# kvignesh1420/rlap

Hardware: AMD Instinct MI355X
Metric: eliminated-vertices/sec (higher is better)
Workload: dtype f64

## Files before the change

__graft_entry__.py:

```python
import os
import subprocess
import sys

ROOT = os.path.dirname(os.path.abspath(__file__))
if ROOT not in sys.path:
    sys.path.insert(0, ROOT)


def build() -> None:
    subprocess.check_call(["make", "-C", os.path.join(ROOT, "rlap_amd", "csrc"), "-s", "ARCH=gfx950"])
    subprocess.check_call(["make", "-C", os.path.join(ROOT, "oracle"), "-s"])
    src = os.path.join(ROOT, "tests", "csrc", "host_mirror.cc")
    so = os.path.join(ROOT, "tests", "csrc", "libhost_mirror.so")
    subprocess.check_call(["g++", "-std=c++17", "-O2", "-msse4.2", "-mavx", "-fPIC", "-shared", "-o", so, src])
    src16 = os.path.join(ROOT, "tests", "csrc", "host_mirror_narrow.cc")
    so16 = os.path.join(ROOT, "tests", "csrc", "libhost_mirror_narrow.so")
    subprocess.check_call(["g++", "-std=c++17", "-O2", "-msse4.2", "-mavx", "-fPIC", "-shared", "-o", so16, src16])
    subprocess.check_call(["gcc", "-std=c99", "-Wall", "-Wextra", "-O1", "-I", os.path.join(ROOT, "include"), "-I", "/opt/rocm/include",
                           os.path.join(ROOT, "examples", "cabi_caller.c"), "-o", os.path.join(ROOT, "examples", "cabi_caller"),
                           "-L", os.path.join(ROOT, "rlap_amd"), "-lrlap_hip", "-L", "/opt/rocm/lib", "-lamdhip64",
                           "-Wl,-rpath,$ORIGIN/../rlap_amd", "-Wl,-rpath,/opt/rocm/lib"])
    import rlap_amd
    from rlap_amd import _lib
    _lib.load()


def smoke() -> None:
    import numpy as np
    import torch
    assert torch.cuda.is_available(), "smoke() needs cuda:0"
    import oracle
    from rlap_amd import graphs, ops
    n = 2000
    ei = graphs.barabasi_albert(n, 8, 1)
    with torch.cuda.device(0):
        out = ops.approximate_cholesky(ei.cuda(), None, n, n // 2, "degree", "asc").numpy()
    ref = oracle.approximate_cholesky(ei.numpy(), None, n, n // 2, "degree", "asc")
    assert out.shape == ref.shape and np.array_equal(out, ref), "HIP path differs from the oracle"
    perm = np.random.RandomState(0).permutation(n)
    with torch.cuda.device(0):
        out2 = ops.approximate_cholesky(ei.cuda(), None, n, n // 2, "random", "asc", perm=torch.from_numpy(perm)).numpy()
    ref2 = oracle.approximate_cholesky(ei.numpy(), None, n, n // 2, "random", "asc", perm=perm)
    assert out2.shape == ref2.shape and np.array_equal(out2, ref2), "HIP path differs from the oracle (o_v=random)"
    print(f"smoke ok: {out.shape[0]} rows bit-exact vs oracle; stats={ops.last_stats}")


if __name__ == "__main__":
    build()
    if len(sys.argv) > 1 and sys.argv[1] == "smoke":
        smoke()
```

rlap_amd/csrc/rlap_core.h:

```cpp
#pragma once
#include <stdint.h>

#if defined(__HIPCC__)
#define RLAP_HD __host__ __device__ __forceinline__
#define RLAP_HD_NOINLINE __host__ __device__ __noinline__
#else
#define RLAP_HD inline
#define RLAP_HD_NOINLINE inline
#endif

namespace rlap {

enum { OV_RANDOM = 0, OV_DEGREE = 1, OV_COARSEN = 2 };
enum { ON_ASC = 0, ON_DESC = 1, ON_RANDOM = 2 };

enum {
    ST_OK = 0,
    ST_NOT_SYMMETRIC = 1,
    ST_INDEX_RANGE = 2,
    ST_BAD_ARG = 3,
    ST_POOL_OVERFLOW = 4,
    ST_LOG_OVERFLOW = 5,
    ST_RNG_OVERFLOW = 6,
    ST_OUT_OVERFLOW = 7,
// ... 471 lines not shown
            for (int32_t j = 0; j < m; ++j) { csum += B.a_val[j]; B.cum[j] = csum; }
            if (A.rng_mode != RNG_COUNTER && G.n_draws >= A.rng_len) return ST_RNG_OVERFLOW;
            double u = arr_uniform(A, G.n_draws, v, 0); G.n_draws += 1;
            double r = u * csum;
            int32_t koff = upper_index(B.cum, m, r);
            int32_t k = B.a_nbr[koff];
            double wk = B.a_val[koff];
            A.e[B.a_twin[koff]].val = 0;
            int32_t xk = B.t_of[koff];
            pq_op(B.t_key[xk], B.t_mv[xk], G.n, -1, len0);
            for (int32_t j = 0; j < m; ++j) {
                if (j == koff) continue;
                pq_op(B.t_key[xk], B.t_mv[xk], G.n, +1, len0 + 1 + j);
                double w = B.a_val[j];
                double nw = (wk * w) / (wk + w);
                int rc = serial_rewire(A, B.a_twin[j], B.a_nbr[j], k, nw);
                if (rc) return rc;
            }
        }
    } else {
        double csum = 0;
        for (int32_t j = 0; j < m; ++j) { csum += B.a_val[j]; B.cum[j] = csum; }
        if (A.rng_mode != RNG_COUNTER && m > 1 && G.n_draws + (m - 1) > A.rng_len) return ST_RNG_OVERFLOW;
        double wdeg = csum, colScale = 1;
        for (int32_t j = 0; j < m - 1; ++j) {
            double w = B.a_val[j] * colScale;
            double f = w / wdeg;
            double u = arr_uniform(A, G.n_draws + j, v, j);
            double r = u * (csum - B.cum[j]) + B.cum[j];
            int32_t koff = upper_index(B.cum, m, r);
            B.ksel[j] = koff;
            double omf = 1 - f;
            B.newv[j] = f * omf * wdeg;
            colScale = colScale * omf;
            wdeg = wdeg * omf * omf;
        }
        if (m > 1) G.n_draws += m - 1;
        for (int32_t j = 0; j < m - 1; ++j) {
            int32_t koff = B.ksel[j];
            if (use_pq) { int32_t xk = B.t_of[koff]; pq_op(B.t_key[xk], B.t_mv[xk], G.n, +1, len0 + j); }
            int rc = serial_rewire(A, B.a_twin[j], B.a_nbr[j], B.a_nbr[koff], B.newv[j]);
            if (rc) return rc;
        }
        if (m > 0) {
            if (use_pq && e1 + 1 < (int64_t)G.n) { int32_t xl = B.t_of[m - 1]; pq_op(B.t_key[xl], B.t_mv[xl], G.n, -1, len0 + m); }
            A.e[B.a_twin[m - 1]].val = 0;
        }
    }
    if (use_pq) return pq_commit_serial(A, G, B, m);
    return ST_OK;
}

RLAP_HD int32_t serial_output(const Arrays& A, const GraphDesc& G, const ColBuf& B, int32_t cap, int32_t v, double* out, int64_t row0, bool count_only) {
    int32_t len0 = serial_gather(A, v, B, cap);
    if (len0 > cap) return -1;
    int32_t m = serial_sort_merge(A, G, B, len0, false, false);
    if (count_only) return m;
    serial_order(A, B, m, v, 1, G.vbase);
    for (int32_t j = 0; j < m; ++j) {
        double* o = out + 3 * (row0 + j);
        o[0] = (double)B.a_nbr[j]; o[1] = (double)v; o[2] = B.a_val[j];
    }
    return m;
}


constexpr int BCAP = 32;

struct TRes {
    int32_t key_after;
    int16_t mv;
    uint8_t c;
    uint8_t flags;
};
struct Ent {
    double val;
    union {
        double aux;
        TRes res;
    };
    int32_t nbr;
    int32_t twin;
};
enum { CF_BIG = 1, CF_DUP = 2, CF_COMPLEX = 4, CF_DEP = 8, CF_TIE = 16, CF_NEQ = 32, CF_READY = 64, CF_PATCHED = 128 };
constexpr int DEPMAX = 4;
enum { TF_CONTENDED = 1 };

template <int BC> struct CandPad {};
template <> struct CandPad<64> { int64_t pad64; };
template <> struct CandPad<128> { int64_t pad128; };
template <int BC>
struct CandT : CandPad<BC> {
    static constexpr int CAP = BC;
    Ent e[BC];
    uint8_t ksel[BC];
    int32_t v;
    int32_t m;
    int32_t flags;
    int32_t src;
    int32_t ndraw;
    int32_t koff;
    int32_t cp1;
    int32_t acnt;
    int32_t ext;
    int32_t nmv;
    int32_t nkill;
    int32_t cb[BC <= 16 ? 2 : (BC <= 32 ? 3 : (BC <= 64 ? 4 : 5))];
    int32_t ndep;
    uint8_t dep[4];
    int64_t draw0;
};
static_assert(sizeof(CandT<16>) == 472 && sizeof(CandT<32>) == 872, "record sizes the LDS budget of the round kernel is counted with");
typedef CandT<BCAP> Cand;

RLAP_HD TRes& ent_tres(Ent& e) { return e.res; }

struct EntLessNbr { RLAP_HD bool operator()(const Ent& x, const Ent& y) const { return x.nbr < y.nbr; } };
struct EntLessVal { RLAP_HD bool operator()(const Ent& x, const Ent& y) const { return x.val < y.val; } };
struct EntGreaterVal { RLAP_HD bool operator()(const Ent& x, const Ent& y) const { return x.val > y.val; } };
struct EntLessAux { RLAP_HD bool operator()(const Ent& x, const Ent& y) const { return x.aux < y.aux; } };

struct KI { double k; uint8_t idx; };
struct KIRef {
    Ent* e; uint8_t* ix; int i;
    RLAP_HD operator KI() const { KI v; v.k = e[i].aux; v.idx = ix[i]; return v; }
    RLAP_HD KIRef& operator=(const KI& v) { e[i].aux = v.k; ix[i] = v.idx; return *this; }
    RLAP_HD KIRef& operator=(const KIRef& o) { KI v = o; e[i].aux = v.k; ix[i] = v.idx; return *this; }
};
struct KIArr {
    Ent* e; uint8_t* ix;
    RLAP_HD KIRef operator[](int i) const { KIRef r; r.e = e; r.ix = ix; r.i = i; return r; }
};
struct KILess { RLAP_HD bool operator()(const KI& x, const KI& y) const { return x.k < y.k; } };
struct KIGreater { RLAP_HD bool operator()(const KI& x, const KI& y) const { return x.k > y.k; } };

template <class CT>
RLAP_HD void cand_order_index(const Arrays& A, CT& C) {
    const int32_t m = C.m;
    for (int32_t j = 0; j < m; ++j) C.ksel[j] = (uint8_t)j;
    KIArr arr; arr.e = C.e; arr.ix = C.ksel;
    if (CT::CAP <= 32) {
        if (A.o_n == ON_DESC && A.o_v != OV_COARSEN) gs_std_sort_small<KI>(arr, m, KIGreater());
        else gs_std_sort_small<KI>(arr, m, KILess());
    } else {
        if (A.o_n == ON_DESC && A.o_v != OV_COARSEN) gs_std_sort<KI>(arr, m, KIGreater());
        else gs_std_sort<KI>(arr, m, KILess());
    }
    C.ndraw = (A.o_v == OV_COARSEN) ? (m >= 1 ? 1 : 0) : (m > 1 ? m - 1 : 0);
}

template <class CT>
RLAP_HD bool cand_merges_multi_edges(const Arrays& A) { return CT::CAP >= 64 && A.o_v == OV_RANDOM; }

template <class CT>
RLAP_HD void cand_meta(const Arrays& A, int32_t v, CT& C) {
    C.v = v; C.flags = 0; C.m = 0; C.ndraw = 0; C.koff = 0; C.nkill = 0; C.nmv = 0; C.ndep = 0;
    int32_t cp0 = A.colptr[v], cp1 = A.colptr[v + 1];
    int32_t acnt = A.vr[v].app_cnt;
    int32_t base = A.vr[v].app_chunk;
    C.cp1 = cp1; C.acnt = acnt; C.ext = (cp1 - cp0) + acnt;
    if (C.ext > CT::CAP) { C.flags = CF_BIG; C.ext = 0; return; }
    if (acnt > 0) {
        int ct = chunk_of(acnt - 1);
        for (int c = ct; c >= 0; --c) { C.cb[c] = base; if (c > 0) base = A.e[base].nbr; }
    }
}
template <class CT>
RLAP_HD int32_t cand_slot(const CT& C, int32_t e) {
    if (e < C.acnt) {
        int32_t a = C.acnt - 1 - e;
        int c = chunk_of(a);
        return C.cb[c] + 1 + (a - chunk_start(c));
    }
    return C.cp1 - 1 - (e - C.acnt);
}
template <class CT>
RLAP_HD void cand_load(const Arrays& A, CT& C, int32_t e) {
    int32_t s = cand_slot(C, e);
    C.e[e].val = A.e[s].val; C.e[e].nbr = A.e[s].nbr; C.e[e].twin = A.e[s].twin; C.e[e].aux = 0;
}
template <class CT>
RLAP_HD void cand_finish(const Arrays& A, CT& C, int32_t vbase = 0) {
    if (C.flags & CF_BIG) return;
    int32_t len = 0;
    for (int32_t e = 0; e < C.ext; ++e) {
        if (C.e[e].val > 0) { if (len != e) C.e[len] = C.e[e]; ++len; }
    }
    C.m = len;
    gs_std_sort<Ent>(C.e, len, EntLessNbr());
    if (cand_merges_multi_edges<CT>(A)) {
        int32_t mm = 0, nk = 0;
        int32_t kill[CT::CAP];
        for (int32_t i = 0; i < len; ++i) {
            if (mm == 0 || C.e[i].nbr != C.e[mm - 1].nbr) { if (mm != i) C.e[mm] = C.e[i]; ++mm; }
            else { C.e[mm - 1].val += C.e[i].val; kill[nk++] = C.e[i].twin; }
        }
        for (int32_t q = 0; q < nk; ++q) C.e[mm + q].twin = kill[q];
        C.nkill = nk;
        len = mm;
        C.m = len;
    } else {
        for (int32_t i = 1; i < len; ++i) if (C.e[i].nbr == C.e[i - 1].nbr) { C.flags = CF_DUP; return; }
    }
    if (A.o_n == ON_RANDOM || A.o_v == OV_COARSEN) {
        uint64_t kb = keyed_order_base(A.shuffle_seed, C.v - vbase, 0);
        for (int32_t i = 0; i < len; ++i) C.e[i].aux = keyed_order_dkey(kb, C.e[i].nbr - vbase);
        gs_std_sort<Ent>(C.e, len, EntLessAux());
    } else if (A.o_n == ON_ASC) {
        gs_std_sort<Ent>(C.e, len, EntLessVal());
    } else {
        gs_std_sort<Ent>(C.e, len, EntGreaterVal());
    }
    C.ndraw = (A.o_v == OV_COARSEN) ? (len >= 1 ? 1 : 0) : (len > 1 ? len - 1 : 0);
}
template <class CT>
RLAP_HD void cand_prepare(const Arrays& A, int32_t v, CT& C, int32_t vbase = 0) {
    cand_meta(A, v, C);
    for (int32_t e = 0; e < C.ext; ++e) cand_load(A, C, e);
    cand_finish(A, C, vbase);
}

template <class CT>
RLAP_HD bool cand_patch(const Arrays& A, CT* cand, int32_t d, int32_t vbase) {
    CT& C = cand[d];
    if (C.nkill > 0) return false;
    for (int32_t q = 0; q < C.ndep; ++q) {
        const int32_t j = C.dep[q];
        const CT& J = cand[j];
        int32_t p = -1;
        for (int32_t z = 0; z < J.m; ++z) if (J.e[z].nbr == C.v) p = z;
        if (p < 0 || p == J.m - 1) return false;
        for (int32_t z = 0; z < J.m - 1; ++z) if (J.ksel[z] == p) return false;
        if (!(J.e[p].val > 0)) return false;
        const int32_t k = J.e[J.ksel[p]].nbr;
        int32_t qd = -1;
        for (int32_t z = 0; z < C.m; ++z) { if (C.e[z].nbr == J.v) qd = z; if (C.e[z].nbr == k) { C.flags |= CF_DUP; return false; } }
        if (qd < 0) return false;
        C.e[qd].nbr = k; C.e[qd].val = J.e[p].val; C.e[qd].twin = ~(j * CT::CAP + p);
    }
    C.flags |= CF_PATCHED;
    const int32_t len = C.m;
    gs_std_sort<Ent>(C.e, len, EntLessNbr());
    if (A.o_n == ON_RANDOM || A.o_v == OV_COARSEN) {
        uint64_t kb = keyed_order_base(A.shuffle_seed, C.v - vbase, 0);
        for (int32_t i = 0; i < len; ++i) C.e[i].aux = keyed_order_dkey(kb, C.e[i].nbr - vbase);
        gs_std_sort<Ent>(C.e, len, EntLessAux());
    } else if (A.o_n == ON_ASC) {
        gs_std_sort<Ent>(C.e, len, EntLessVal());
    } else {
        gs_std_sort<Ent>(C.e, len, EntGreaterVal());
    }
    return true;
}

RLAP_HD int32_t ent_upper_index(const Ent* e, int32_t m, double r) {
    int32_t lo = 0, hi = m;
    while (lo < hi) {
        int32_t mid = (lo + hi) >> 1;
        if (e[mid].aux > r) hi = mid; else lo = mid + 1;
    }
    return lo < m ? lo : m - 1;
}

template <class CT>
RLAP_HD void cand_cumsum(const Arrays& A, CT& C) {
    const int32_t m = C.m;
    double csum = 0;
    for (int32_t j = 0; j < m; ++j) { csum += C.e[j].val; C.e[j].aux = csum; }
    if (A.o_v == OV_COARSEN && m >= 1) {
        double u = arr_uniform(A, C.draw0, C.v, 0);
        double r = u * csum;
        int32_t koff = ent_upper_index(C.e, m, r);
        C.koff = koff;
        double wk = C.e[koff].val;
        for (int32_t j = 0; j < m; ++j) {
            if (j == koff) continue;
            double w = C.e[j].val;
            C.e[j].val = (wk * w) / (wk + w);
            C.ksel[j] = (uint8_t)koff;
        }
    }
}
template <class CT>
RLAP_HD void cand_pick(const Arrays& A, CT& C, int32_t j) {
    const int32_t m = C.m;
    double csum = C.e[m - 1].aux;
    double u = arr_uniform(A, C.draw0 + j, C.v, j);
    double cj = C.e[j].aux;
    double r = u * (csum - cj) + cj;
    C.ksel[j] = (uint8_t)ent_upper_index(C.e, m, r);
}
template <class CT>
RLAP_HD void cand_recur(const Arrays& A, CT& C) {
    if (A.o_v == OV_COARSEN) return;
    const int32_t m = C.m;
    if (m < 1) return;
    double wdeg = C.e[m - 1].aux, colScale = 1;
    for (int32_t j = 0; j < m - 1; ++j) {
        double w = C.e[j].val * colScale;
        double f = w / wdeg;
        double omf = 1 - f;
// ... 88 lines not shown
```

rlap_amd/csrc/rlap_kernels.hip:

```cpp
#include <hip/hip_runtime.h>
#include <stdint.h>
#include <cstdlib>
#include <type_traits>

#include "rlap_core.h"
#include "rlap_kernels.h"
#include "rlap_wave_sort.h"

namespace rlap {


#ifndef RLAP_ELIM_PQ_TU
__global__ __launch_bounds__(320) void k_mt19937_64_table(double* __restrict__ out, int64_t count) {
    constexpr int NN = 312, MM = 156;
    constexpr uint64_t MATRIX_A = 0xB5026F5AA96619E9ull, UM = 0xFFFFFFFF80000000ull, LM = 0x7FFFFFFFull;
    __shared__ uint64_t x[NN];
    const int tid = threadIdx.x;
    if (tid == 0) {
        uint64_t s = 5489ull;
        x[0] = s;
        for (int i = 1; i < NN; ++i) { s = 6364136223846793005ull * (s ^ (s >> 62)) + (uint64_t)i; x[i] = s; }
    }
    __syncthreads();
    for (int64_t base = 0; base < count; base += NN) {
// ... 863 lines not shown
        __hip_atomic_store(&help[0], 4, __ATOMIC_RELAXED, __HIP_MEMORY_SCOPE_WORKGROUP);
    }
#define BIG_HELP_FINISH() do { if (helped) { if (lane == 0) { int _sp = 0; while (__hip_atomic_load(&help[0], __ATOMIC_RELAXED, __HIP_MEMORY_SCOPE_WORKGROUP) != 2 && ++_sp < SPIN_LIMIT) __builtin_amdgcn_s_sleep(1); \
        if (_sp >= SPIN_LIMIT) G.status = ST_INTERNAL; \
        __hip_atomic_store(&help[0], 0, __ATOMIC_RELAXED, __HIP_MEMORY_SCOPE_WORKGROUP); } __builtin_amdgcn_fence(__ATOMIC_ACQUIRE, "workgroup"); WAVE_SYNC(); } \
        else if (lane == 0) __hip_atomic_store(&help[0], 3, __ATOMIC_RELAXED, __HIP_MEMORY_SCOPE_WORKGROUP); } while (0)
    if (lane == 0) {
        double csum = 0;
        for (int j = 0; j < m; ++j) { csum += cum[j]; cum[j] = csum; }
        if (!helped) {
            double wdeg = csum, colScale = 1;
            for (int j = 0; j < m - 1; ++j) {
                double w = newv[j] * colScale;
                double f = w / wdeg;
                double omf = 1 - f;
                newv[j] = f * omf * wdeg;
                colScale = colScale * omf;
                wdeg = wdeg * omf * omf;
            }
        }
    }
    WAVE_SYNC();
    const double csum = m > 0 ? cum[m - 1] : 0.0;
    const int64_t draws0 = G.n_draws;
    const int ndraw = m > 1 ? m - 1 : 0;
    if (draws0 + ndraw > A.rng_len) { BIG_HELP_FINISH(); if (lane == 0) G.status = ST_RNG_OVERFLOW; WAVE_SYNC(); return true; }

    for (int j = lane; j < m - 1; j += 64) {
        double u = arr_uniform(A, draws0 + j, v, j);
        double cj = cum[j];
        double r = u * (csum - cj) + cj;
        B.ksel[j] = upper_index(cum, m, r);
    }
    WAVE_SYNC();

    BIG_HELP_FINISH();
#undef BIG_HELP_FINISH
    int32_t status = 0;
    for (int j0 = 0; j0 < m - 1; j0 += 64) {
        const int j = j0 + lane;
        const bool act = j < m - 1;
        const int32_t ks = act ? B.ksel[j] : 0;
        const int32_t k = act ? B.a_nbr[ks] : -1;
        uint64_t mymask = __ballot(act);
        static_assert(BIGE <= 8192, "13 bits of target position");
#pragma unroll
        for (int bit = 0; bit < 13; ++bit) {
            const bool mybit = (ks >> bit) & 1;
            const uint64_t bb = __ballot(act && mybit);
            mymask &= mybit ? bb : ~bb;
        }
        if (act && lane == __builtin_ctzll(mymask)) {
            int32_t a = ld_agent(&A.vr[k].app_cnt), chunk = ld_agent(&A.vr[k].app_chunk);
            uint64_t mm = mymask;
            while (mm) { const int l = __builtin_ctzll(mm); mm &= mm - 1; L.tmp[l] = alloc_in_column(A, a, chunk, &status); }
            A.vr[k].app_cnt = a; A.vr[k].app_chunk = chunk;
        }
        __threadfence();
        WAVE_SYNC();
        if (act && status == 0) {
            const int32_t s_r = B.a_twin[j], s_n = L.tmp[lane];
            const double nw = newv[j];
            A.e[s_r].nbr = k; A.e[s_r].val = nw; A.e[s_r].twin = s_n;
            A.e[s_n].nbr = B.a_nbr[j]; A.e[s_n].val = nw; A.e[s_n].twin = s_r;
        }
        WAVE_SYNC();
        if (__ballot(status != 0) != 0ull) break;
    }
    if (__ballot(status != 0) != 0ull) { if (lane == 0) G.status = ST_POOL_OVERFLOW; WAVE_SYNC(); return true; }
    if (lane == 0) {
        if (m >= 1) A.e[B.a_twin[m - 1]].val = 0;
        G.n_draws = draws0 + ndraw;
    }
    WAVE_SYNC();
    return true;
}


constexpr int PASSES = 4;

struct CRec { int32_t x, i, j; };
constexpr int batch_ccap(int BC, int NTT) { return BC == 16 ? NTT / 4 : NTT / 2; }

template <int BC, int NTT>
struct BatchLdsT {
    CandT<BC> cand[4 * NTT / BC];
    union {
        struct {
            uint64_t mkey[NTT];
            int32_t mval[NTT];
            int32_t hidx[NTT];
        };
        int32_t hcnt[4 * NTT];
    };
    int32_t pslot[4 * NTT];
    unsigned long long cmask[4 * NTT / BC];
    CRec cont[batch_ccap(BC, NTT)];
    CRec csorted[batch_ccap(BC, NTT)];
    int32_t scan[NTT / 64 + 8];
};

template <int BC, int NTT>
union ElimSharedT {
    BatchLdsT<BC, NTT> b;
    ElimLdsT<(NTT >= 1024 ? ECAP : ECAP_SMALL)> e;
    BigElimLdsT<(NTT >= 1024 ? 7168 : 1536)> g;
};
static_assert(sizeof(ElimSharedT<64, 1024>) == sizeof(BatchLdsT<64, 1024>) && sizeof(ElimSharedT<32, 1024>) == sizeof(BatchLdsT<32, 1024>) &&
              sizeof(ElimSharedT<16, 1024>) == sizeof(BatchLdsT<16, 1024>),
              "the single-vertex paths borrow the batch round's LDS");

template <int NWAVE>
__device__ __noinline__ int block_excl_scan(int val, int* scratch, int* total) {
    const int tid = threadIdx.x, lane = tid & 63, wave = tid >> 6;
    int incl = val;
    for (int off = 1; off < 64; off <<= 1) { int t = __shfl_up(incl, off); if (lane >= off) incl += t; }
    if (lane == 63) scratch[wave] = incl;
    __syncthreads();
    int base = 0, tot = 0;
    for (int w = 0; w < NWAVE; ++w) { int sw = scratch[w]; if (w < wave) base += sw; tot += sw; }
    __syncthreads();
    *total = tot;
    return base + incl - val;
}

template <int NWAVE>
__device__ __forceinline__ int block_rank(bool flag, int* scratch, int* total) {
    return block_excl_scan<NWAVE>(flag ? 1 : 0, scratch, total);
}


__device__ __forceinline__ void rewire_store(const Arrays& A, int32_t s_r, int32_t s_n, int32_t nbr_j, int32_t k, double nw) {
    Slot a; a.val = nw; a.nbr = k; a.twin = s_n;
    Slot b; b.val = nw; b.nbr = nbr_j; b.twin = s_r;
    A.e[s_r] = a;
    A.e[s_n] = b;
}

template <class CT>
__device__ __forceinline__ void push_into_target(const Arrays& A, const CT& C, int32_t j, int32_t& a, int32_t& chunk, int32_t* status) {
    const int32_t x = C.e[j].nbr;
    if (A.o_v == OV_COARSEN) {
        if (j != C.koff) return;
        for (int32_t p = 0; p < C.m; ++p) {
            if (p == C.koff) continue;
            int32_t s_n = alloc_in_column(A, a, chunk, status);
            if (*status) return;
            rewire_store(A, C.e[p].twin, s_n, C.e[p].nbr, x, C.e[p].val);
        }
    } else {
        for (int32_t p = 0; p < C.m - 1; ++p) {
            if (C.ksel[p] != j) continue;
            int32_t s_n = alloc_in_column(A, a, chunk, status);
            if (*status) return;
            rewire_store(A, C.e[p].twin, s_n, C.e[p].nbr, x, C.e[p].val);
        }
    }
}

template <class CT>
__device__ __forceinline__ void slots_into_target(const Arrays& A, const CT& C, int32_t j, int32_t& a, int32_t& chunk, int32_t* status, int32_t* pslot_row) {
    const bool co = A.o_v == OV_COARSEN;
    if (co && j != C.koff) return;
    const int32_t plast = co ? C.m : C.m - 1;
    for (int32_t p = 0; p < plast; ++p) {
        if (co ? (p == C.koff) : (C.ksel[p] != j)) continue;
        pslot_row[p] = alloc_in_column(A, a, chunk, status);
        if (*status) return;
    }
// ... 281 lines not shown
        wave_bitonic128(ok2, os2, lane, m);
        bool anytie;
        {
            unsigned long long pv0 = __shfl_up(ok2[0], 1), pv1 = __shfl_up(ok2[1], 1);
            const unsigned long long edge = __shfl(ok2[0], 63);
            if (lane == 0) pv1 = edge;
            anytie = (__ballot(c0 && lane > 0 && ok2[0] == pv0) | __ballot(c1 && ok2[1] == pv1)) != 0ull;
        }
        if (m <= 16 || !anytie) {
            if (c0) C.ksel[lane] = (uint8_t)os2[0];
            if (c1) C.ksel[64 + lane] = (uint8_t)os2[1];
        } else {
            bool ok;
            if (m <= 64) {
                double key = k0;
                int idx = lane, pos = lane;
                ok = desc ? wave_sort64<true>(key, idx, m, lane, tmp64, &pos) : wave_sort64<false>(key, idx, m, lane, tmp64, &pos);
                if (ok && lane < m) C.ksel[pos] = (uint8_t)idx;
            } else {
                if (c0) rec[lane] = (uint16_t)lane;
                if (c1) rec[64 + lane] = (uint16_t)(64 + lane);
                WAVE_SYNC();
                ok = desc ? wave_lvl_sort<uint16_t, WideAuxGreater, 2>(rec, m, WideAuxGreater{C.e}, ulist, dlist, tab, tab2, lane)
                          : wave_lvl_sort<uint16_t, WideAuxLess, 2>(rec, m, WideAuxLess{C.e}, ulist, dlist, tab, tab2, lane);
                if (ok) { if (c0) C.ksel[lane] = (uint8_t)rec[lane]; if (c1) C.ksel[64 + lane] = (uint8_t)rec[64 + lane]; }
            }
            WAVE_SYNC();
            if (!ok && lane == 0) cand_order_index_call(A, C);
        }
    }
    WAVE_SYNC();
    double pv0 = 0, pv1 = 0; int32_t pn0 = 0, pn1 = 0, pt0 = 0, pt1 = 0;
    if (c0) { const Ent& Sx = C.e[C.ksel[lane]]; pv0 = Sx.val; pn0 = Sx.nbr; pt0 = Sx.twin; }
    if (c1) { const Ent& Sx = C.e[C.ksel[64 + lane]]; pv1 = Sx.val; pn1 = Sx.nbr; pt1 = Sx.twin; }
    WAVE_SYNC();
    if (c0) { Ent& E = C.e[lane]; E.val = pv0; E.nbr = pn0; E.twin = pt0; E.aux = 0; }
    if (c1) { Ent& E = C.e[64 + lane]; E.val = pv1; E.nbr = pn1; E.twin = pt1; E.aux = 0; }
    if (lane == 0) C.ndraw = (A.o_v == OV_COARSEN) ? 1 : (m > 1 ? m - 1 : 0);
    WAVE_SYNC();
}

__device__ __noinline__ void serial_eliminate_call(const Arrays& A, GraphDesc& G, const ElimScratch& S, int32_t v0, int64_t e1) {
    ColBuf Bf = S.colbuf(G.scr_base);
    int rc = serial_eliminate(A, G, Bf, G.scr_cap, v0, e1);
    if (rc) G.status = rc;
}

template <int BC>
__device__ __forceinline__ uint64_t group_pick_mask(const uint8_t* ksel, int32_t m, bool cand_ok, int lane) {
    static_assert(BC == 32 || BC == 64, "one candidate per (half-)wave");
    constexpr int BITS = BC == 32 ? 5 : 6;
    const int gl = lane & (BC - 1), hb = lane & (64 - BC);
    const bool vp = cand_ok && gl < m - 1;
    const int t = vp ? (int)ksel[gl] : 0;
    uint64_t mm = __ballot(vp);
#pragma unroll
    for (int b = 0; b < BITS; ++b) {
        const uint64_t bb = __ballot(vp && ((t >> b) & 1));
        mm &= ((gl >> b) & 1) ? bb : ~bb;
    }
    return (mm >> hb) & (BC == 64 ? ~0ull : 0xFFFFFFFFull);
}

template <int OV, int ON, int BC, int NTT>
__global__ __launch_bounds__(NTT, (NTT >= 1024 ? 1 : 4)) void k_eliminate_batch_t(Arrays A_in, GraphDesc* __restrict__ gd, ElimScratch S,
                                                           int32_t* __restrict__ batch_pos, const int32_t* __restrict__ in_flags,
                                                           const double* __restrict__ in_acc) {
    constexpr int NT = NTT;
    uint32_t jit_ctr = 0;
#define BSYNC() do { __syncthreads(); if (S.jitter > 0) { ++jit_ctr; if (((((uint32_t)threadIdx.x >> 6) * 2654435761u + jit_ctr * 40503u) >> 7 & 3u) == 0u) \
        for (int _q = 0; _q < S.jitter; ++_q) __builtin_amdgcn_s_sleep(8); } } while (0)
    constexpr int NWAVE = NT / 64;
    constexpr int SLOTS = PASSES * NT;
    constexpr int MCAP = NT;
    constexpr int CCAP = batch_ccap(BC, NTT);
    constexpr bool NARROW = (BC == 16);
    static_assert(!NARROW || (OV == OV_DEGREE && NTT == 1024), "the 16-slot shape exists for the degree order, 1024 threads");
    constexpr int SEQSH = NARROW ? 6 : 8;
    static_assert(((SLOTS / BC - 1) << SEQSH | ((1 << SEQSH) - 1)) <= 0x7FFF && (BC > 32 || 2 * BC < (1 << SEQSH)), "(candidate, op) fits 15 bits");
    constexpr int HBITS = (SLOTS == 4096) ? 12 : (SLOTS == 2048) ? 11 : 10;
    static_assert((1 << HBITS) == SLOTS, "hash table = one place per slot");
    constexpr int BCAP = BC;
    constexpr int BATCH = SLOTS / BC;
    typedef CandT<BC> Cand;
    typedef BatchLdsT<BC, NTT> BatchLds;
    constexpr bool MERGE = (BC >= 64 && OV == OV_RANDOM);
    constexpr bool PATCH = (OV == OV_DEGREE);
    constexpr int GSH = BC >= 64 ? 0 : 64 - BC;
    constexpr uint64_t GMASK = BC >= 64 ? ~0ull : ((1ull << (BC & 63)) - 1ull);
    Arrays A = A_in;
    A.o_v = OV;
    A.o_n = ON;
    A.shuffle_seed = A_in.shuffle_seed + (uint64_t)blockIdx.x;
    A.vbase = gd[blockIdx.x].vbase;
    __shared__ ElimSharedT<BC, NTT> sh;
    __shared__ GraphDesc G;
    __shared__ int32_t s_help[3];
    __shared__ int32_t s_nc, s_pmax, s_p, s_ncont, s_nmoves, s_status, s_nhigh, s_nlow, s_pool_cur, s_pool_end, s_anydep, s_npatched;
    __shared__ int32_t s_dirb;
    __shared__ int32_t s_dir[BDIR];
    constexpr int32_t POOL_GRAB = NT >= 1024 ? POOL_GRAB_BIG : POOL_GRAB_SMALL;
    constexpr bool EQG = NTT < 1024 || BC == 128 || NARROW;
    constexpr int EC1 = NTT >= 1024 ? ECAP : ECAP_SMALL;
    __shared__ uint8_t s_eqperm[EQG ? 1 : BC - 16][EQG ? 1 : BC];
    __shared__ uint8_t s_eqinv[EQG ? 1 : BC - 16][EQG ? 1 : BC];
    const uint8_t* __restrict__ eqg = S.eqtab + (BC == 64 ? 0 : (BC == 128 ? EQTAB_OFF128 : EQTAB_OFF32));
    BatchLds& L = sh.b;
    const int g = blockIdx.x;
    const int tid = threadIdx.x;
    if (S.poison >= 0) {
        uint32_t* const w = reinterpret_cast<uint32_t*>(&sh);
        const uint32_t pat = 0x01010101u * (uint32_t)(S.poison & 0xFF);
        for (size_t q = tid; q < sizeof(sh) / 4; q += NT) w[q] = pat;
        BSYNC();
    }
    if (tid == 0) {
        G = gd[g]; s_nc = 0; s_pmax = BATCH + 1; s_p = BATCH + 1; s_ncont = 0; s_nmoves = 0; s_pool_cur = 0; s_pool_end = 0; s_anydep = 0; s_npatched = 0;
        s_help[0] = 0; s_help[1] = 0; s_help[2] = 0; s_dirb = -1;
        if (G.resume) { s_pool_cur = G.pool_cur; s_pool_end = G.pool_end; }
        int32_t bad = 0;
        if (in_flags[FLAG_RANGE]) bad = ST_INDEX_RANGE;
        else if (in_flags[FLAG_CROSS] || in_flags[FLAG_PERM]) bad = ST_BAD_ARG;
        else if (in_acc[2] != 0.0 || !(in_acc[0] <= 1e-24 * in_acc[1])) bad = ST_NOT_SYMMETRIC;
        s_status = bad;
    }
    if constexpr (!EQG) {
        for (int base = 0; base < BC - 16; base += BATCH) {
            const int row = base + tid;
            if (tid < BATCH && row < BC - 16) {
                Cand& C = L.cand[tid];
                const int nn = 17 + row;
                for (int q = 0; q < nn; ++q) { C.e[q].aux = 1.0; C.ksel[q] = (uint8_t)q; }
                C.m = nn;
                Arrays A3 = A;
                cand_order_index_call(A3, C);
                for (int q = 0; q < BC; ++q) s_eqperm[row][q] = q < nn ? C.ksel[q] : (uint8_t)q;
                for (int q = 0; q < BC; ++q) s_eqinv[row][s_eqperm[row][q]] = (uint8_t)q;
            }
        }
    }
    BSYNC();
    const int32_t n = G.n;
    const bool use_pq = A.o_v != OV_RANDOM;
    int64_t nelim = G.t < (int64_t)(n - 1) ? G.t : (int64_t)(n - 1);
    if (nelim < 0 || s_status != 0) nelim = 0;
    int64_t done = 0;
    int32_t rounds = 0, singles = 0;
    if (G.resume) {
        done = G.n_elim; rounds = G.pad0; singles = G.pad1;
        if (G.status != 0 || nelim < done) nelim = done;
        if (NARROW && G.narrow) nelim = done;
    }
    const int32_t rounds_in = rounds, singles_in = singles;
    bool handover = false;
    bool pending_long = false;
    long long t_prev = 0;
    __shared__ long long s_prof[40];
#define PHASE_STAMP(k) do { if (S.prof && tid == 0 && g == 0) { long long _t = wall_clock64(); s_prof[k] += _t - t_prev; t_prev = _t; } } while (0)
    long long clk0 = 0, wall0 = 0;
    if (S.prof && tid == 0 && g == 0) { for (int q = 0; q < 40; ++q) s_prof[q] = 0; t_prev = wall_clock64(); clk0 = clock64(); wall0 = t_prev; }

    while (done < nelim) {
        int tid_round = threadIdx.x;
        asm volatile("" : "+v"(tid_round));
        const int tid = tid_round;
        const int lane = tid & 63;
        constexpr bool GROUPED = (BC == 64);
// ... 29 lines not shown
        }
        ++rounds;
        const int32_t bcap = NARROW ? (S.narrow_batch < BATCH ? S.narrow_batch : BATCH) : BATCH;
        const int32_t Bcur = (int32_t)((nelim - done) < (int64_t)bcap ? (nelim - done) : (int64_t)bcap);
        int32_t b = 0;
        if (use_pq) {
            while (true) {
                b = G.bucket_base + G.minlist;
                const int32_t cnt = A.bs_cnt[b];
                int32_t oc0 = A.ocur[b];
                const int32_t oe = A.oend[b];
                if (s_dirb != b) {
                    if (tid < BDIR) s_dir[tid] = A.bs_dir[(int64_t)b * BDIR + tid];
                    BSYNC();
                    if (tid == 0) s_dirb = b;
                }
                int32_t top = cnt;
                while (s_nc < Bcur && (top > 0 || oc0 < oe)) {
                    const int32_t a = top - 1 - tid;
                    bool vs = false, vo = false;
                    int32_t v_s = -1, v_o = -1;
                    if (a >= 0) {
                        const int cdir = bs_chunk_of(a);
                        const int32_t sl = s_dir[cdir] + (a - bs_chunk_start(cdir));
                        v_s = A.bs_v[sl];
                        vs = (A.vr[v_s].pqpos == A.bs_id[sl]);
                    }
                    const bool last_stack = top <= NT;
                    const int32_t oc = oc0 + tid;
                    if (last_stack && oc < oe) { v_o = A.orig_order[oc]; vo = (A.vr[v_o].pqpos == -1); }
                    int tot;
                    const int r = block_excl_scan<NWAVE>((vs ? 1 : 0) | (vo ? (1 << 16) : 0), L.scan, &tot);
                    const int rs = r & 0xFFFF, ro = r >> 16, ts = tot & 0xFFFF, to = tot >> 16;
                    const int base = s_nc;
                    BSYNC();
                    if (vs && base + rs < Bcur) { L.cand[base + rs].v = v_s; L.cand[base + rs].src = a; }
                    if (vo && base + ts + ro < Bcur) { L.cand[base + ts + ro].v = v_o; L.cand[base + ts + ro].src = ~oc; }
                    if (tid == 0) s_nc = (base + ts + to < Bcur) ? base + ts + to : Bcur;
                    BSYNC();
                    top = top > NT ? top - NT : 0;
                    if (last_stack) oc0 += NT;
                }
                if (s_nc > 0) break;
                BSYNC();
                if (tid == 0) {
                    A.bs_cnt[b] = 0; A.ocur[b] = oe;
                    G.minlist += 1;
                    if (G.minlist > 2 * n) s_status = ST_INTERNAL;
                }
                BSYNC();
                if (s_status) break;
            }
            if (s_status) break;
        } else {
            if (tid < Bcur) { L.cand[tid].v = G.vbase + (int32_t)A.perm[G.vbase + n - (done + tid + 1)]; L.cand[tid].src = 0; }
            if (tid == 0) s_nc = Bcur;
            BSYNC();
        }
        const int32_t nc = s_nc;
        PHASE_STAMP(0);

        if (tid < nc) {
            int32_t v = L.cand[tid].v, src = L.cand[tid].src;
            cand_meta(A, v, L.cand[tid]);
            L.cand[tid].src = src;
            batch_pos[v] = tid;
            if (L.cand[tid].flags & CF_BIG) atomicMin(&s_pmax, tid);
        }
        BSYNC();
        const bool first_is_big = (L.cand[0].flags & CF_BIG) != 0;
        if constexpr (NARROW) {
            if (first_is_big) {
                if (tid < nc) batch_pos[L.cand[tid].v] = -1;
                --rounds;
                handover = true;
                break;
            }
        }
        if (!first_is_big) {
            static_assert(BATCH * BCAP == PASSES * NT && (BC == 16 || BC == 32 || BC == 64 || BC == 128), "slot loops are unrolled for PASSES passes");
            auto SI = [&](int k) -> int32_t { return BC == 128 ? ((k >> 1) * NWAVE + (tid >> 6)) : (k * NT + tid) / BCAP; };
            auto SE = [&](int k) -> int32_t { return BC == 128 ? (((k & 1) << 6) + (tid & 63)) : (k * NT + tid) % BCAP; };
            double lv[PASSES]; int32_t ln[PASSES], lt[PASSES]; bool la[PASSES];
            const int32_t cut0 = (OV == OV_RANDOM) ? s_pmax : nc;
#pragma unroll
            for (int k = 0; k < PASSES; ++k) {
                const int32_t i = SI(k), e = SE(k);
                la[k] = (i < nc) && (OV != OV_RANDOM || i < cut0) && (e < L.cand[i].ext);
                lv[k] = 0; ln[k] = 0; lt[k] = 0;
                if (la[k]) {
                    int32_t sl = cand_slot(L.cand[i], e);
                    const Slot g = A.e[sl]; lv[k] = g.val; ln[k] = g.nbr; lt[k] = g.twin;
                }
            }
            int32_t bpk[PASSES];
#pragma unroll
            for (int k = 0; k < PASSES; ++k) { bpk[k] = -1; if (la[k] && lv[k] > 0) bpk[k] = batch_pos[ln[k]]; }
            const bool keyed = (A.o_n == ON_RANDOM || A.o_v == OV_COARSEN);
            bool ready[PASSES];
#pragma unroll
            for (int k = 0; k < PASSES; ++k) ready[k] = false;
            if constexpr (BC <= 64) {
#pragma unroll
            for (int k = 0; k < PASSES; ++k) {
                const int32_t idx = k * NT + tid;
                const int32_t i = idx / BCAP, e = idx % BCAP;
                const int hb = lane & GSH;
                const bool live = la[k] && lv[k] > 0;
                const uint64_t half = (__ballot(live) >> hb) & GMASK;
                const int32_t nxt = __shfl_down(ln[k], 1);
                const bool cand_ok = (i < nc) && (OV != OV_RANDOM || i < cut0) && !(L.cand[i].flags & CF_BIG);
                const int32_t ext = cand_ok ? L.cand[i].ext : 0;
                const bool unsorted = la[k] && (e + 1 < ext) && !(ln[k] > nxt);
                const uint64_t hbad = (__ballot(unsorted) >> hb) & GMASK;
                const int f = half ? __builtin_ctzll(half) : 0;
                const double w0 = __shfl(lv[k], hb + f);
                const uint64_t hdw = (__ballot(live && lv[k] != w0) >> hb) & GMASK;
                ready[k] = cand_ok && !keyed && L.cand[i].acnt == 0 && hbad == 0 && hdw == 0;
                if (ready[k]) {
                    Cand& C = L.cand[i];
                    const int32_t m = __popcll(half);
                    if (live) {
                        const int32_t r = __popcll(half & ~((2ull << e) - 1ull));
                        const int32_t pos = (NARROW || m <= 16) ? r : (int32_t)(EQG ? eqg[(BC - 16) * BC + (m - 17) * BC + r] : s_eqinv[EQG ? 0 : m - 17][EQG ? 0 : r]);
                        Ent& E = C.e[pos];
                        E.val = lv[k]; E.nbr = ln[k]; E.twin = lt[k]; E.aux = 0;
                    }
                    if (e == 0) {
                        C.m = m;
                        C.ndraw = m > 1 ? m - 1 : 0;
                        C.flags |= CF_READY;
                    }
                    la[k] = false;
                }
            }
            }
#pragma unroll
            for (int k = 0; k < PASSES; ++k) {
                if (la[k]) {
                    Ent& E = L.cand[SI(k)].e[SE(k)];
                    E.val = lv[k]; E.nbr = ln[k];
                }
            }
#pragma unroll
            for (int k = 0; k < PASSES; ++k) {
                const int32_t i = SI(k);
                if (bpk[k] >= 0 && bpk[k] < i) {
                    if (PATCH) {
                        const int32_t q = atomicAdd(&L.cand[i].ndep, 1);
                        if (q < DEPMAX) L.cand[i].dep[q] = (uint8_t)bpk[k]; else atomicMin(&s_pmax, i);
                        s_anydep = 1;
                    } else atomicMin(&s_pmax, i);
                }
            }
            if (tid < nc && (L.cand[tid].flags & CF_BIG)) atomicMin(&s_pmax, tid);
            BSYNC();
            const int32_t ncp = s_pmax < nc ? s_pmax : nc;
#pragma unroll
            for (int k = 0; k < PASSES; ++k) if (SI(k) >= ncp) { la[k] = false; ready[k] = false; }
            PHASE_STAMP(9);
            if constexpr (BC == 128) {
                uint8_t* const wscr = reinterpret_cast<uint8_t*>(L.hcnt) + (size_t)(tid >> 6) * WIDE_SCR_BYTES;
                static_assert((size_t)NWAVE * WIDE_SCR_BYTES <= sizeof(int32_t) * 8 * (size_t)NT, "scratch of the waves fits hcnt + pslot");
#pragma unroll
                for (int cc = 0; cc < PASSES / 2; ++cc) {
                    const int32_t i = cc * NWAVE + (tid >> 6);
                    if (i < ncp && !(L.cand[i].flags & CF_BIG)) {
                        cand_prepare_wide(A.o_v, A.o_n, A.shuffle_seed, L.cand[i], G.vbase, lv[2 * cc], ln[2 * cc], lt[2 * cc], la[2 * cc], lv[2 * cc + 1], ln[2 * cc + 1], lt[2 * cc + 1], la[2 * cc + 1], wscr, eqg);
                    }
                }
            } else {
            int32_t rk[PASSES];
            bool merge_k[PASSES];
#pragma unroll
            for (int k = 0; k < PASSES; ++k) {
                rk[k] = -1; merge_k[k] = false;
                if (__ballot(la[k]) == 0ull) continue;
                const int32_t idx = k * NT + tid;
                const int32_t i = idx / BCAP, e = idx % BCAP;
                const bool live = la[k] && lv[k] > 0;
                const uint64_t half = (__ballot(live) >> (lane & GSH)) & GMASK;
                const int32_t nxt = __shfl_down(ln[k], 1);
                const bool unsorted = la[k] && (i < ncp) && (e + 1 < L.cand[i].ext) && !(ln[k] > nxt);
                const uint64_t hbad = (__ballot(unsorted) >> (lane & GSH)) & GMASK;
                rk[k] = -1;
                if (!ready[k] && i < ncp && L.cand[i].ext > 0) {
                    Cand& C = L.cand[i];
                    if (C.acnt == 0 && hbad == 0) {
                        if (live) rk[k] = __popcll(half & ~((2ull << e) - 1ull));
                        if (e == 0) C.m = __popcll(half);
                    } else if (!MERGE) {
                        uint32_t skey = live ? (uint32_t)ln[k] : 0x7FFFFFFFu;
                        int ssrc = e;
#pragma unroll
                        for (int kk = 2; kk <= BC; kk <<= 1) {
#pragma unroll
                            for (int jj = kk >> 1; jj > 0; jj >>= 1) {
                                const uint32_t okey = (uint32_t)__shfl_xor((int)skey, jj);
                                const int osrc = __shfl_xor(ssrc, jj);
                                const bool keep_min = (((e & jj) == 0) == ((e & kk) == 0));
                                const bool other_less = okey < skey || (okey == skey && osrc < ssrc);
                                if (keep_min == other_less) { skey = okey; ssrc = osrc; }
                            }
                        }
                        const uint32_t pkey = (uint32_t)__shfl_up((int)skey, 1);
                        const bool dupp = e > 0 && skey == pkey && skey != 0x7FFFFFFFu;
                        const int myrank = __builtin_amdgcn_ds_permute(((lane & GSH) + ssrc) << 2, e);
                        if (__ballot(dupp) >> (lane & GSH) & GMASK) { if (e == 0) atomicOr(&C.flags, CF_DUP); }
                        if (live) rk[k] = myrank;
                        if (e == 0) C.m = __popcll(half);
                    } else {
                        const int32_t ext = C.ext, me = ln[k];
                        int32_t r = 0, eqb = 0;
                        bool dup = false;
                        if (live) {
                            for (int32_t q = 0; q < ext; ++q) {
                                bool lq = C.e[q].val > 0;
                                int32_t nq = C.e[q].nbr;
                                r += (lq && nq < me) ? 1 : 0;
                                eqb += (lq && nq == me && q < e) ? 1 : 0;
                                dup |= (lq && nq == me && q != e);
                            }
                        }
                        const int32_t nlive = __popcll(half);
                        const bool anydup = __ballot(live && dup) != 0ull;
                        if (!anydup) {
                            if (live) rk[k] = r;
                        } else if (nlive <= 16) {
                            if (live) rk[k] = r + eqb;
                            merge_k[k] = true;
                        } else {
                            int32_t* tmp = L.pslot + (tid >> 6) * 256;
                            if (live) tmp[144 + __popcll(half & lanemask_lt(lane))] = lane;
                            WAVE_SYNC();
                            const int src = lane < nlive ? tmp[144 + lane] : 0;
                            double key = (double)__shfl(me, src);
                            int idx = src, pos = lane;
                            const WS64 wr = wave_sort64_call<false>(key, idx, nlive, lane, tmp);
                            key = wr.key; idx = wr.idx; pos = wr.pos;
                            const bool ok = wr.ok != 0;
                            WAVE_SYNC();
                            if (lane < nlive) tmp[144 + idx] = pos;
                            WAVE_SYNC();
                            if (ok) { if (live) rk[k] = tmp[144 + lane]; merge_k[k] = true; }
                            else if (lane == 0) atomicOr(&C.flags, CF_DUP);
                            WAVE_SYNC();
                        }
                        if (lane == 0) C.m = nlive;
                    }
                }
            }
            WAVE_SYNC();
            PHASE_STAMP(12);
#pragma unroll
            for (int k = 0; k < PASSES; ++k) {
                if (__ballot(rk[k] >= 0) == 0ull) continue;
                if (rk[k] >= 0) {
                    const int32_t idx = k * NT + tid;
                    Cand& C = L.cand[idx / BCAP];
                    Ent& E = C.e[rk[k]];
                    E.val = lv[k]; E.nbr = ln[k]; E.twin = lt[k];
                    E.aux = keyed ? keyed_order_dkey(keyed_order_base(A.shuffle_seed, C.v - G.vbase, 0), ln[k] - G.vbase) : lv[k];
                }
            }
            if (MERGE) {
#pragma unroll
                for (int k = 0; k < PASSES; ++k) {
                    if (!merge_k[k]) continue;
                    WAVE_SYNC();
                    Cand& C = L.cand[k * NWAVE + (tid >> 6)];
                    const int32_t nl = C.m;
// ... 1909 lines not shown
```

Measured before the change: 1.939 million.

## Let narrow 16-slot candidates accept up to 32 slots when live entries fit

The narrow (BC=16) round kernel now lets a candidate take up to 32 stored slots. It loads a second half of entries and compacts the live (positive-weight) ones into the 16-entry record, marking them unsorted when order is broken. Candidates whose stored columns exceed 16 but hold mostly dead entries can be eliminated in the fast batched path instead of being flagged big and handed to a slower path. In exchange it adds extra global loads, ballots and wave syncs, and a round is abandoned with a handover when the first candidate overflows.

After: 1.947 million, median of 6. No clear change (+0.4%).

```diff
diff --git a/__graft_entry__.py b/__graft_entry__.py
--- a/__graft_entry__.py
+++ b/__graft_entry__.py
@@ -16,6 +16,9 @@
     src16 = os.path.join(ROOT, "tests", "csrc", "host_mirror_narrow.cc")
     so16 = os.path.join(ROOT, "tests", "csrc", "libhost_mirror_narrow.so")
     subprocess.check_call(["g++", "-std=c++17", "-O2", "-msse4.2", "-mavx", "-fPIC", "-shared", "-o", so16, src16])
+    srcl = os.path.join(ROOT, "tests", "csrc", "host_mirror_live16.cc")
+    sol = os.path.join(ROOT, "tests", "csrc", "libhost_mirror_live16.so")
+    subprocess.check_call(["g++", "-std=c++17", "-O2", "-msse4.2", "-mavx", "-fPIC", "-shared", "-o", sol, srcl])
     subprocess.check_call(["gcc", "-std=c99", "-Wall", "-Wextra", "-O1", "-I", os.path.join(ROOT, "include"), "-I", "/opt/rocm/include",
                            os.path.join(ROOT, "examples", "cabi_caller.c"), "-o", os.path.join(ROOT, "examples", "cabi_caller"),
                            "-L", os.path.join(ROOT, "rlap_amd"), "-lrlap_hip", "-L", "/opt/rocm/lib", "-lamdhip64",
diff --git a/rlap_amd/csrc/rlap_core.h b/rlap_amd/csrc/rlap_core.h
--- a/rlap_amd/csrc/rlap_core.h
+++ b/rlap_amd/csrc/rlap_core.h
@@ -577,16 +577,19 @@
     int32_t nbr;
     int32_t twin;
 };
-enum { CF_BIG = 1, CF_DUP = 2, CF_COMPLEX = 4, CF_DEP = 8, CF_TIE = 16, CF_NEQ = 32, CF_READY = 64, CF_PATCHED = 128 };
+enum { CF_BIG = 1, CF_DUP = 2, CF_COMPLEX = 4, CF_DEP = 8, CF_TIE = 16, CF_NEQ = 32, CF_READY = 64, CF_PATCHED = 128,
+       CF_UNSORTED = 256 };
 constexpr int DEPMAX = 4;
 enum { TF_CONTENDED = 1 };
 
 template <int BC> struct CandPad {};
 template <> struct CandPad<64> { int64_t pad64; };
 template <> struct CandPad<128> { int64_t pad128; };
-template <int BC>
+template <int BC, int SC = BC>
 struct CandT : CandPad<BC> {
     static constexpr int CAP = BC;
+    static constexpr int SLOTCAP = SC;
+    static_assert(SC >= BC, "every live entry is a slot");
     Ent e[BC];
     uint8_t ksel[BC];
     int32_t v;
@@ -600,12 +603,14 @@
     int32_t ext;
     int32_t nmv;
     int32_t nkill;
-    int32_t cb[BC <= 16 ? 2 : (BC <= 32 ? 3 : (BC <= 64 ? 4 : 5))];
+    int32_t cb[SC <= 16 ? 2 : (SC <= 32 ? 3 : (SC <= 64 ? 4 : (SC <= 128 ? 5 : 6)))];
+    static_assert(SC <= 256, "chunk bases are counted up to 256 slots");
     int32_t ndep;
     uint8_t dep[4];
     int64_t draw0;
 };
 static_assert(sizeof(CandT<16>) == 472 && sizeof(CandT<32>) == 872, "record sizes the LDS budget of the round kernel is counted with");
+static_assert(sizeof(CandT<16, 32>) == 472, "the third chunk base of the two-capacity record takes the padding in front of draw0");
 typedef CandT<BCAP> Cand;
 
 RLAP_HD TRes& ent_tres(Ent& e) { return e.res; }
@@ -654,7 +659,7 @@
     int32_t acnt = A.vr[v].app_cnt;
     int32_t base = A.vr[v].app_chunk;
     C.cp1 = cp1; C.acnt = acnt; C.ext = (cp1 - cp0) + acnt;
-    if (C.ext > CT::CAP) { C.flags = CF_BIG; C.ext = 0; return; }
+    if (C.ext > CT::SLOTCAP) { C.flags = CF_BIG; C.ext = 0; return; }
     if (acnt > 0) {
         int ct = chunk_of(acnt - 1);
         for (int c = ct; c >= 0; --c) { C.cb[c] = base; if (c > 0) base = A.e[base].nbr; }
@@ -711,7 +716,20 @@
 template <class CT>
 RLAP_HD void cand_prepare(const Arrays& A, int32_t v, CT& C, int32_t vbase = 0) {
     cand_meta(A, v, C);
-    for (int32_t e = 0; e < C.ext; ++e) cand_load(A, C, e);
+    if (CT::SLOTCAP > CT::CAP) {
+        if (C.flags & CF_BIG) return;
+        int32_t len = 0;
+        for (int32_t e = 0; e < C.ext; ++e) {
+            const int32_t s = cand_slot(C, e);
+            if (!(A.e[s].val > 0)) continue;
+            if (len == CT::CAP) { C.flags = CF_BIG; C.ext = 0; return; }
+            C.e[len].val = A.e[s].val; C.e[len].nbr = A.e[s].nbr; C.e[len].twin = A.e[s].twin; C.e[len].aux = 0;
+            ++len;
+        }
+        C.ext = len;
+    } else {
+        for (int32_t e = 0; e < C.ext; ++e) cand_load(A, C, e);
+    }
     cand_finish(A, C, vbase);
 }
 
diff --git a/rlap_amd/csrc/rlap_kernels.hip b/rlap_amd/csrc/rlap_kernels.hip
--- a/rlap_amd/csrc/rlap_kernels.hip
+++ b/rlap_amd/csrc/rlap_kernels.hip
@@ -969,9 +969,11 @@
 struct CRec { int32_t x, i, j; };
 constexpr int batch_ccap(int BC, int NTT) { return BC == 16 ? NTT / 4 : NTT / 2; }
 
+template <int BC> using RoundCandT = CandT<BC, (BC == 16 ? 32 : BC)>;
+
 template <int BC, int NTT>
 struct BatchLdsT {
-    CandT<BC> cand[4 * NTT / BC];
+    RoundCandT<BC> cand[4 * NTT / BC];
     union {
         struct {
             uint64_t mkey[NTT];
@@ -1419,7 +1421,7 @@
     static_assert((1 << HBITS) == SLOTS, "hash table = one place per slot");
     constexpr int BCAP = BC;
     constexpr int BATCH = SLOTS / BC;
-    typedef CandT<BC> Cand;
+    typedef RoundCandT<BC> Cand;
     typedef BatchLdsT<BC, NTT> BatchLds;
     constexpr bool MERGE = (BC >= 64 && OV == OV_RANDOM);
     constexpr bool PATCH = (OV == OV_DEGREE);
@@ -1615,6 +1617,8 @@
             auto SI = [&](int k) -> int32_t { return BC == 128 ? ((k >> 1) * NWAVE + (tid >> 6)) : (k * NT + tid) / BCAP; };
             auto SE = [&](int k) -> int32_t { return BC == 128 ? (((k & 1) << 6) + (tid & 63)) : (k * NT + tid) % BCAP; };
             double lv[PASSES]; int32_t ln[PASSES], lt[PASSES]; bool la[PASSES];
+            constexpr int PB = NARROW ? PASSES : 1;
+            double lvB[PB]; int32_t lnB[PB], ltB[PB]; bool laB[PB];
             const int32_t cut0 = (OV == OV_RANDOM) ? s_pmax : nc;
 #pragma unroll
             for (int k = 0; k < PASSES; ++k) {
@@ -1624,6 +1628,50 @@
                 if (la[k]) {
                     int32_t sl = cand_slot(L.cand[i], e);
                     const Slot g = A.e[sl]; lv[k] = g.val; ln[k] = g.nbr; lt[k] = g.twin;
+                }
+                if constexpr (NARROW) {
+                    laB[k] = (i < nc) && (e + 16 < L.cand[i].ext);
+                    lvB[k] = 0; lnB[k] = 0; ltB[k] = 0;
+                    if (laB[k]) {
+                        int32_t sl = cand_slot(L.cand[i], e + 16);
+                        const Slot g = A.e[sl]; lvB[k] = g.val; lnB[k] = g.nbr; ltB[k] = g.twin;
+                    }
+                }
+            }
+            if constexpr (NARROW) {
+#pragma unroll
+                for (int k = 0; k < PASSES; ++k) {
+                    const int32_t i = SI(k), e = SE(k);
+                    const int32_t ext = (i < nc) ? L.cand[i].ext : 0;
+                    const bool wide = ext > 16;
+                    if (__ballot(wide) == 0ull) continue;
+                    const int hb = lane & GSH;
+                    const bool liveA = la[k] && lv[k] > 0, liveB = laB[k] && lvB[k] > 0;
+                    const uint32_t mA = (uint32_t)((__ballot(liveA) >> hb) & GMASK), mB = (uint32_t)((__ballot(liveB) >> hb) & GMASK);
+                    const int32_t nxtA = __shfl_down(ln[k], 1), nxtB = __shfl_down(lnB[k], 1), firstB = __shfl(lnB[k], hb);
+                    const bool badA = la[k] && !(ln[k] > (e == 15 ? firstB : nxtA));
+                    const bool badB = laB[k] && (e + 17 < ext) && !(lnB[k] > nxtB);
+                    const bool anybad = ((__ballot(wide && (badA || badB)) >> hb) & GMASK) != 0ull;
+                    const int32_t nA = __popc(mA), nlive = nA + __popc(mB);
+                    const bool fits = nlive <= 16;
+                    if (wide && fits) {
+                        Cand& C = L.cand[i];
+                        const uint32_t below = (1u << e) - 1u;
+                        if (liveA) { Ent& E = C.e[__popc(mA & below)]; E.val = lv[k]; E.nbr = ln[k]; E.twin = lt[k]; }
+                        if (liveB) { Ent& E = C.e[nA + __popc(mB & below)]; E.val = lvB[k]; E.nbr = lnB[k]; E.twin = ltB[k]; }
+                    }
+                    WAVE_SYNC();
+                    if (wide) {
+                        Cand& C = L.cand[i];
+                        la[k] = fits && e < nlive;
+                        lv[k] = 0; ln[k] = 0; lt[k] = 0;
+                        if (la[k]) { const Ent& E = C.e[e]; lv[k] = E.val; ln[k] = E.nbr; lt[k] = E.twin; }
+                        if (e == 0) {
+                            if (fits) { C.ext = nlive; if (anybad) C.flags |= CF_UNSORTED; }
+                            else { C.flags = CF_BIG; C.ext = 0; atomicMin(&s_pmax, i); }
+                        }
+                    }
+                    WAVE_SYNC();
                 }
             }
             int32_t bpk[PASSES];
@@ -1649,7 +1697,7 @@
                 const int f = half ? __builtin_ctzll(half) : 0;
                 const double w0 = __shfl(lv[k], hb + f);
                 const uint64_t hdw = (__ballot(live && lv[k] != w0) >> hb) & GMASK;
-                ready[k] = cand_ok && !keyed && L.cand[i].acnt == 0 && hbad == 0 && hdw == 0;
+                ready[k] = cand_ok && !keyed && L.cand[i].acnt == 0 && hbad == 0 && hdw == 0 && !(NARROW && (L.cand[i].flags & CF_UNSORTED));
                 if (ready[k]) {
                     Cand& C = L.cand[i];
                     const int32_t m = __popcll(half);
@@ -1688,6 +1736,14 @@
             }
             if (tid < nc && (L.cand[tid].flags & CF_BIG)) atomicMin(&s_pmax, tid);
             BSYNC();
+            if constexpr (NARROW) {
+                if (L.cand[0].flags & CF_BIG) {
+                    if (tid < nc) batch_pos[L.cand[tid].v] = -1;
+                    --rounds;
+                    handover = true;
+                    break;
+                }
+            }
             const int32_t ncp = s_pmax < nc ? s_pmax : nc;
 #pragma unroll
             for (int k = 0; k < PASSES; ++k) if (SI(k) >= ncp) { la[k] = false; ready[k] = false; }
@@ -1719,7 +1775,7 @@
                 rk[k] = -1;
                 if (!ready[k] && i < ncp && L.cand[i].ext > 0) {
                     Cand& C = L.cand[i];
-                    if (C.acnt == 0 && hbad == 0) {
+                    if (C.acnt == 0 && hbad == 0 && !(NARROW && (C.flags & CF_UNSORTED))) {
                         if (live) rk[k] = __popcll(half & ~((2ull << e) - 1ull));
                         if (e == 0) C.m = __popcll(half);
                     } else if (!MERGE) {
```
